# wjakob/nori

Hardware: AMD Instinct MI355X
Metric: Mrays/sec (primary+secondary) at 1024x1024 256spp (higher is better)
Workload: dtype f32; 1 GPU; pa4-cbox-path_mis; generator=tests/golden/pa4-cbox-path_mis.npz (scenes/pa4/cbox/cbox-distributed.xml), integrator=path_mis, width=1024, height=1024, spp=256, triangles=7948, parallelism=single GPU, seed_mode=per_sample, engine=wavefront

## Files before the change

### nori_amd/csrc/device/wavefront.hip

```cpp
#include <hip/hip_runtime.h>

#include <algorithm>
#include <cstdio>
#include <cstdlib>
#include <string>
#include <type_traits>
#include <vector>

#ifdef NORI_LAB
#include "wf_experiments.h"
#else
#define NORI_EXP_Q_GLOBAL
#define NORI_EXP_Q_LDS
#define NORI_EXP_Q_ALU
#define NORI_PROF_DECL
#define NORI_PROF_MARK(acc)
#define NORI_PROF_STORE
#define NORI_PROF_REPORT(h, k)
#define NORI_LAB_SHADE_PAD
#define NORI_LAB_SHADE_VERTEX
#define NORI_LAB_SHADE_STORE
#endif

#include "film.h"
#include "ktimer.h"
#include "shade_tables.h"
#include "rt_path.h"
#include "wavefront.h"
#include "wf_records.h"

using namespace nrt;

namespace {

constexpr int kB = 256;

enum { C_N = 0, C_HEAD = 2, C_OVERFLOW = 4, C_TAIL_HEAD = 5, C_SAMPLE = 6, C_HEAD_FRESH = 8, C_COUNT = 12 };
enum { S_CAM = 0, S_CLOSEST = 1, S_SHADOW = 2, S_NODES = 3, S_TRIS = 4, S_INVALID = 5, S_COUNT = 8 };
enum { Z_TRIPS = 0, Z_INNER_TRIPS = 1, Z_INNER_LANES = 2, Z_LEAF_TRIPS = 3, Z_LEAF_LANES = 4, Z_REFILLS = 5, Z_REFILL_LANES = 6, Z_COUNT = 8 };

constexpr uint32_t kShadeChunk = 4096u;

struct WfState {
    P3 *o;
    f4 *dA;
    f4 *dB;
    f4 *T_eta, *L_pdf;
    P3 *Ld;
    uint32_t *sidx;
    unsigned long long *rng;
};

struct WfBuf {
    WfState st[2];
    f4 *hit;
    f2 *samp_pos;
    P3 *samp_L;
    uint32_t *ctr;
    unsigned long long *stats;
    uint32_t capacity;
    int *stack_spill;
    unsigned long long *census;
};

struct WfBatch {
    uint32_t tile_first, n_tiles;
    uint32_t s_first, n_spp;
    uint32_t tile_mod, tile_rem, tiles_x;
    int32_t tile_w;
    int32_t inner_repeat;
    uint32_t flags;
    uint32_t pool;
};

enum { kStoredOnly = 0, kFreshOnly = 1, kMixed = 2 };
struct PassShape { uint32_t n_s, s0, n_fresh, n_f0, n; };
template <int MODE> __device__ __forceinline__ PassShape pass_shape(const uint32_t *ctr, int cur, const WfBatch &bt) {
    PassShape ps;
    ps.n_s = ctr[C_N + cur];
    ps.s0 = ctr[C_SAMPLE + cur];
    ps.n_f0 = (ps.n_s + 255u) & ~255u;
    const uint32_t total = bt.n_tiles * 256u * bt.n_spp;
    ps.n_fresh = MODE == kStoredOnly ? 0u : min(total - ps.s0, bt.pool > ps.n_f0 ? bt.pool - ps.n_f0 : 0u);
    ps.n = ps.n_fresh ? ps.n_f0 + ps.n_fresh : ps.n_s;
    return ps;
}
constexpr uint32_t kBatchNoAsmLoop = 1u;
constexpr uint32_t kBatchCountQ = 2u;

template <int DEPTH, bool SPILL, int BLOCK = kB>
struct LdsStackW {
    int *base; int sp;
    int *spill; uint32_t spill_stride;
    __device__ __forceinline__ void init(char *smem, int *spill_, uint32_t stride_) {
        base = reinterpret_cast<int *>(smem) + threadIdx.x; sp = 0; spill = spill_; spill_stride = stride_;
    }
    __device__ __forceinline__ void reset() { sp = 0; }
    __device__ __forceinline__ void push(int v) {
        if (sp < DEPTH) base[sp * BLOCK] = v;
        else spill[(size_t) (sp - DEPTH) * spill_stride + blockIdx.x * BLOCK + threadIdx.x] = v;
        sp++;
    }
    __device__ __forceinline__ int pop_or(int empty_value) {
        if (sp == 0) return empty_value;
        sp--;
        if (sp < DEPTH) return base[sp * BLOCK];
        return spill[(size_t) (sp - DEPTH) * spill_stride + blockIdx.x * BLOCK + threadIdx.x];
    }
    static constexpr int kLdsEntries = DEPTH;
};

typedef __attribute__((address_space(3))) int lds_int_t;
__device__ __forceinline__ uint32_t lds_address(const void *generic) {
    return (uint32_t) reinterpret_cast<uintptr_t>((const __attribute__((address_space(3))) char *) generic);
}
__device__ __forceinline__ lds_int_t *lds_int_at(uint32_t address) { return reinterpret_cast<lds_int_t *>(address); }

template <int DEPTH, int BLOCK>
struct LdsStackW<DEPTH, false, BLOCK> {
    uint32_t top;
    uint32_t wave_base;
    __device__ __forceinline__ void init(char *smem, int *, uint32_t) {
        wave_base = (uint32_t) __builtin_amdgcn_readfirstlane((int) (lds_address(smem) + (threadIdx.x & ~63u) * 4u)); top = 0u;
    }
    __device__ __forceinline__ void reset() {
        uint32_t lane;
        asm volatile("v_mbcnt_lo_u32_b32 %0, -1, 0\n\tv_mbcnt_hi_u32_b32 %0, -1, %0" : "=v"(lane));
        const uint32_t base = wave_base + lane * 4u;
        *lds_int_at(base) = kTravDone; top = base + BLOCK * 4u;
    }
    __device__ __forceinline__ void push(int v) { *lds_int_at(top) = v; top += BLOCK * 4u; }
    __device__ __forceinline__ int pop_or(int) { top -= BLOCK * 4u; return *lds_int_at(top); }
    static constexpr int kLdsEntries = DEPTH + 1;
};
// ... 319 lines not shown
                }
            }
            chunk_pos += min(avail, (uint32_t) __popcll(fresh));
            nClosest += (uint32_t) __popcll(__ballot(startedA));
            if (kFresh) nCam += (uint32_t) __popcll(__ballot(startedCam));
            if (kStored) nShadow += (uint32_t) __popcll(__ballot(startedB));
        }
        if (__ballot(trav_active(tv)) == 0ull) {
            if (exhausted && __ballot((rid & 2u) != 0u) == 0ull) break;
            continue;
        }
        NORI_PROF_MARK(prof_refill)
        if (COUNT) zc[Z_TRIPS]++;
        if constexpr (ASM) {
            static_assert(!WIDE && !COUNT, "the hand-written node loop: BVH2 nodes as 32-B records");
            f3 qo = tv.o, qr = tv.rcp;
            asm volatile("" : "+v"(qo.x), "+v"(qo.y), "+v"(qo.z), "+v"(qr.x), "+v"(qr.y), "+v"(qr.z));
            NodeqRay R;
            nodeq_ray(sc.grid, qo, qr, R);
            uint32_t stack_limit = 0xffffffffu;
            if constexpr (SPILL) stack_limit = stack.limit;
            const bool full = bvh2q_node_loop_asm<BLOCK * 4, SPILL>(tv.node, stack.top, tv.hit.t, R, (int) f2u(qr.x) >> 31, (int) f2u(qr.y) >> 31, (int) f2u(qr.z) >> 31,
                                           sc.nodes_q, image_address, bt.inner_repeat, leaf_threshold,
                                           (!exhausted || __ballot((rid & 2u) != 0u) != 0ull) ? 64 - refill_threshold : -1, stack_limit);
            if (SPILL && full && trav_at_inner(tv)) trav_inner_step_q<false>(sc, stack, tv, tc, top_lds);
        } else
        do {
            if (COUNT) { const int ni = __popcll(__ballot(trav_at_inner(tv))); if (ni) { zc[Z_INNER_TRIPS]++; zc[Z_INNER_LANES] += (uint32_t) ni; } }
            if (trav_at_inner(tv)) {
                if (WIDE) trav_wide_step<COUNT>(sc, stack, tv, tc, top_lds);
                else if (COUNT && count_q) trav_inner_step_q<COUNT>(sc, stack, tv, tc, top_lds);
                else trav_inner_step<COUNT>(sc, stack, tv, tc, top_lds);
            }
        } while (__popcll(__ballot(trav_at_inner(tv))) >= bt.inner_repeat);
        NORI_PROF_MARK(prof_node)
        const bool atLeaf = trav_at_leaf(tv);
        const int nLeaf = __popcll(__ballot(atLeaf));
        const bool innerLeft = __ballot(trav_at_inner(tv)) != 0ull;
        if (COUNT && nLeaf && (nLeaf >= leaf_threshold || !innerLeft)) { zc[Z_LEAF_TRIPS]++; zc[Z_LEAF_LANES] += (uint32_t) nLeaf; }
        if (atLeaf && (nLeaf >= leaf_threshold || !innerLeft)) trav_leaf_step<COUNT, false>(sc, stack, tv, tc, top_lds);
        NORI_PROF_MARK(prof_leaf)
    }
    if (unsaved) st_f4<1>(&b.hit[rid >> 2], tv.any ? hit_pack_here(nullptr, tv.hit.tri != kNoHit) : hit_pack_here(&tv.hit, (rid & 1u) != 0u));
#ifdef NORI_LAB_WAVE_COUNTERS
    if (lane == 0) {
        if (nClosest) atomicAdd(&b.stats[S_CLOSEST], (unsigned long long) nClosest);
        if (nShadow) atomicAdd(&b.stats[S_SHADOW], (unsigned long long) nShadow);
        if (kFresh && nCam) atomicAdd(&b.stats[S_CAM], (unsigned long long) nCam);
    }
#else
    __syncthreads();
    uint32_t *s_sum = reinterpret_cast<uint32_t *>(smem);
    if (threadIdx.x < 4u) s_sum[threadIdx.x] = 0u;
    __syncthreads();
    if (lane == 0) {
        if (nClosest) atomicAdd(&s_sum[0], nClosest);
        if (nShadow) atomicAdd(&s_sum[1], nShadow);
        if (kFresh && nCam) atomicAdd(&s_sum[2], nCam);
    }
    __syncthreads();
    if (threadIdx.x == 0) {
        if (s_sum[0]) atomicAdd(&b.stats[S_CLOSEST], (unsigned long long) s_sum[0]);
        if (s_sum[1]) atomicAdd(&b.stats[S_SHADOW], (unsigned long long) s_sum[1]);
        if (kFresh && s_sum[2]) atomicAdd(&b.stats[S_CAM], (unsigned long long) s_sum[2]);
    }
#endif
    if (COUNT) for (int off = 32; off > 0; off >>= 1) { tc.nodes += (uint32_t) __shfl_down((int) tc.nodes, off); tc.tris += (uint32_t) __shfl_down((int) tc.tris, off); }
    if (lane == 0) {
        if (COUNT) { atomicAdd(&b.stats[S_NODES], (unsigned long long) tc.nodes); atomicAdd(&b.stats[S_TRIS], (unsigned long long) tc.tris); }
        NORI_PROF_STORE
        if (COUNT && b.census) for (int k = 0; k < Z_COUNT; ++k) if (zc[k]) atomicAdd(&b.census[k], (unsigned long long) zc[k]);
    }
}

constexpr int kSB = 256;
static_assert(kSB == 256, "pass_shape starts the new paths of a pass at a multiple of 256");

__device__ __forceinline__ void shade_barrier() { asm volatile("s_waitcnt lgkmcnt(0)\n\ts_barrier" ::: "memory"); }

template <bool LDSTAB> struct ShadeTab { typedef SceneTables type; static __device__ __forceinline__ type make(const DevScene &sc, uint4 *) { type t = {&sc}; return t; } };
template <> struct ShadeTab<true> { typedef LdsTables type; static __device__ __forceinline__ type make(const DevScene &sc, uint4 *s_tab) { return shade_tables_copy(sc, s_tab); } };


#ifndef NORI_SHADE_WGS
#define NORI_SHADE_WGS 4
#endif
template <int INTEG, int MODE, bool LDSTAB, int MATSET>
__global__ __launch_bounds__(kSB, NORI_SHADE_WGS) void wf_shade(DevScene sc, WfBuf b, int cur, WfBatch bt) {
    NORI_LAB_SHADE_PAD
    const WfState S = b.st[cur], D = b.st[cur ^ 1];
    const uint32_t s_first = bt.s_first, n_spp = bt.n_spp;
    __shared__ uint4 s_tab[LDSTAB ? kShadeTabWords / 4 : 1];
    const typename ShadeTab<LDSTAB>::type tab = ShadeTab<LDSTAB>::make(sc, s_tab);
    constexpr bool kFresh = MODE != kStoredOnly, kStored = MODE != kFreshOnly;
    const PassShape shape = pass_shape<MODE>(b.ctr, cur, bt);
    const uint32_t n = shape.n, n_s = shape.n_s;
    const uint32_t rounds_total = (n + kSB - 1) / kSB;
    const uint32_t rounds_per_block = (rounds_total + gridDim.x - 1) / gridDim.x;
    const uint32_t r0 = blockIdx.x * rounds_per_block, r1 = min(rounds_total, r0 + rounds_per_block);
    const uint32_t r_mid = kStored ? min(r1, max(r0, shape.n_f0 / kSB)) : r0;
    __shared__ uint32_t s_wcnt[2][4], s_newbase;
    uint32_t out_base = 0u, out_used = 0u, out_len = 0u;
    bool overflow = false;
    const int wave = (int) (threadIdx.x >> 6), lane = lane_id();
    const uint32_t per_tile = 256u * n_spp;
    uint32_t pf_sidx = 0u; f4 pf_d, pf_L, pf_h;
    pf_d.x = pf_d.y = pf_d.z = pf_d.w = 0.0f; pf_L = pf_h = pf_d;
    auto round = [&](auto fresh_tag, uint32_t r, uint32_t r_end) {
        constexpr bool FRESH = decltype(fresh_tag)::value;
        const uint32_t i = r * kSB + threadIdx.x;
        bool survive = false;
        const uint32_t c_sidx = pf_sidx; const f4 c_d = pf_d, c_L = pf_L, c_h = pf_h;
        if (!FRESH && r + 1u < r_end && i + kSB < n_s) {
            pf_d = ld_f4<2>(&S.dA[i + kSB]); pf_sidx = ld_w<2>(&S.sidx[i + kSB]); pf_L = ld_f4<2>(&S.L_pdf[i + kSB]); pf_h = ld_f4<1>(&b.hit[i + kSB]);
        }
        f4 n_o, n_dA, n_dB, n_T, n_L, n_Ld;
        uint32_t n_fl = 0u, sidx = 0u;
        unsigned long long n_rng = 0ull;
        if (FRESH ? i < n : i < n_s) {
            uint32_t fl; f4 L4, d4, t4; Rng rng0; rng0.state = 0; rng0.inc = 0;
            if (FRESH) {
                f2 ps; RayIn cam;
                sidx = shape.s0 + (i - shape.n_f0);
                fl = first_vertex(sc, bt, sidx, ps, cam, rng0) ? (F_HAS_A | (2u << 4)) : 0u;
                L4.x = L4.y = L4.z = L4.w = 0.0f;
                t4.x = t4.y = t4.z = t4.w = 1.0f;
                d4.x = cam.d.x; d4.y = cam.d.y; d4.z = cam.d.z; d4.w = 0.0f;
            } else {
                d4 = c_d;
                fl = state_flags(d4);
            }
            if (fl & (F_HAS_A | F_HAS_B)) {
                if (!FRESH) { sidx = c_sidx; L4 = c_L; }
                const f4 h = FRESH ? ld_f4<1>(&b.hit[i]) : c_h;
                const uint32_t hw = __float_as_uint(h.w);
                bool done = false;
                NORI_LAB_SHADE_VERTEX
                if (fl & F_HAS_B) {
                    if (!(hw & kOccludedB)) {
                        const P3 ld = ld_p3<2>(&S.Ld[i]);
                        L4.x = L4.x + ld.x; L4.y = L4.y + ld.y; L4.z = L4.z + ld.z;
                    }
                    if (fl & F_END_AFTER_B) done = true;
                }
                PathState st;
                st.L = mk3(L4.x, L4.y, L4.z);
                if (!done) {
                    if (!FRESH) t4 = ld_f4<2>(&S.T_eta[i]);
                    Hit hit; bool found;
                    hit_unpack(sc, h, hit, found);
                    const uint32_t sl = (sidx % per_tile) >> 8;
                    uint64_t rng_state = rng0.state;
                    if (!FRESH) rng_state = ld_w<2>(&S.rng[i]);
                    vertex_unpack(st, fl, L4, t4, rng_state, ((uint64_t) (s_first + sl) << 1u) | 1u);
                    done = path_on_closest<INTEG, typename ShadeTab<LDSTAB>::type, MATSET>(sc, tab, st, hit, found, mk3(d4.x, d4.y, d4.z));
                    if (!done) {
                        survive = true;
                        vertex_pack(st, n_o, n_dA, n_dB, n_T, n_L, n_Ld, n_fl);
                        n_rng = st.rng.state;
                    }
                }
                if (done) {
                    P3 out; out.x = st.L.x; out.y = st.L.y; out.z = st.L.z;
                    st_p3<2>(&b.samp_L[sidx], out);
                }
            }
        }
        const unsigned long long mask = __ballot(survive);
        if (lane == 0) s_wcnt[r & 1u][wave] = (uint32_t) __popcll(mask);
        shade_barrier();
        const uint32_t c0 = s_wcnt[r & 1u][0], c1 = kSB > 64 ? s_wcnt[r & 1u][1] : 0u, c2 = kSB > 128 ? s_wcnt[r & 1u][2] : 0u, c3 = kSB > 192 ? s_wcnt[r & 1u][3] : 0u;
        const uint32_t c = c0 + c1 + c2 + c3;
        uint32_t off = (uint32_t) __popcll(mask & ((1ull << lane) - 1ull));
        off += wave > 0 ? c0 : 0u; off += wave > 1 ? c1 : 0u; off += wave > 2 ? c2 : 0u;
        const uint32_t room = out_len - out_used;
        uint32_t new_base = 0u, want = 0u;
        if (c > room) {
            const uint32_t expect = c * (r1 - r);
            want = r + 1u == r1 ? c - room : min(kShadeChunk, max(c - room, ((expect + expect / 8u + 63u) & ~63u) - min(room, expect)));
            if (threadIdx.x == 0) s_newbase = atomicAdd(&b.ctr[C_N + (cur ^ 1)], want);
            shade_barrier();
            new_base = s_newbase;
            if (new_base + want > b.capacity) overflow = true;
        }
        if (survive && !overflow) {
            const uint32_t j = off < room ? out_base + out_used + off : new_base + (off - room);
            st_p3<2>(&D.o[j], p3_of(n_o)); st_f4<2>(&D.T_eta[j], n_T); st_f4<2>(&D.L_pdf[j], n_L);
            st_f4<2>(&D.dA[j], state_dA(n_dA, n_fl, (n_fl & F_HAS_A) != 0u)); st_w<2>(&D.rng[j], n_rng); st_w<2>(&D.sidx[j], sidx);
            if (n_fl & F_HAS_B) { st_f4<2>(&D.dB[j], n_dB); st_p3<2>(&D.Ld[j], p3_of(n_Ld)); }
            NORI_LAB_SHADE_STORE
        }
        if (c > room) { out_base = new_base; out_used = c - room; out_len = want; }
        else out_used += c;
    };
    if (kStored) {
        if (r0 < r_mid && r0 * kSB + threadIdx.x < n_s) {
            const uint32_t i0 = r0 * kSB + threadIdx.x;
            pf_d = ld_f4<2>(&S.dA[i0]); pf_sidx = ld_w<2>(&S.sidx[i0]); pf_L = ld_f4<2>(&S.L_pdf[i0]); pf_h = ld_f4<1>(&b.hit[i0]);
        }
        for (uint32_t r = r0; r < r_mid; ++r) round(std::false_type(), r, r_mid);
    }
    if (kFresh) for (uint32_t r = r_mid; r < r1; ++r) round(std::true_type(), r, r1);
    for (uint32_t k = out_used + threadIdx.x; k < out_len; k += kSB) { f4 z; z.x = z.y = z.z = z.w = 0.0f; D.dA[out_base + k] = z; }
    if (overflow && threadIdx.x == 0) b.ctr[C_OVERFLOW] = 1u;
}

template <int INTEG, int MATSET = kAnyBsdf>
__global__ __launch_bounds__(kB) void wf_finish(DevScene sc, WfBuf b, int cur, WfBatch bt, int count) {
    extern __shared__ __attribute__((aligned(16))) char smem[];
    LdsStackW<16, true> stack;
    stack.init(smem, b.stack_spill, gridDim.x * kB);
    __shared__ uint4 s_tab[kShadeTabWords / 4];
    shade_tables_to_lds(sc, s_tab);
    const WfState S = b.st[cur];
    const uint32_t n = b.ctr[C_N + cur];
    const uint32_t per_tile = 256u * bt.n_spp;
    uint32_t nClosest = 0, nShadow = 0;
    TraversalCounters tc; tc.nodes = 0; tc.tris = 0;
    bool have = false, dry = false;
    uint32_t sidx = 0u, fl = 0u;
    f4 o, dA, dB, T, L, Ld;
    o.x = o.y = o.z = o.w = 0.0f; dA = dB = T = L = Ld = o;
    unsigned long long rng_state = 0ull;
    while (true) {
        const unsigned long long want = __ballot(!have && !dry);
        if (want != 0ull) {
            uint32_t base = 0u;
            if (lane_id() == 0) base = atomicAdd(&b.ctr[C_TAIL_HEAD], (uint32_t) __popcll(want));
            base = (uint32_t) __builtin_amdgcn_readfirstlane((int) base);
            const uint32_t i = base + __builtin_amdgcn_mbcnt_hi((uint32_t) (want >> 32), __builtin_amdgcn_mbcnt_lo((uint32_t) want, 0u));
            if (!have && !dry) {
                if (i >= n) dry = true;
                else {
                    dA = S.dA[i];
                    fl = state_flags(dA);
                    if (fl & (F_HAS_A | F_HAS_B)) {
                        have = true;
                        sidx = S.sidx[i]; dB = S.dB[i]; T = S.T_eta[i]; L = S.L_pdf[i];
                        const P3 o3 = S.o[i], l3 = S.Ld[i];
                        o.x = o3.x; o.y = o3.y; o.z = o3.z; o.w = kStoredMint; Ld.x = l3.x; Ld.y = l3.y; Ld.z = l3.z; Ld.w = 0.0f;
                        dA.w = kInf;
                        rng_state = S.rng[i];
                    }
                }
            }
        }
        if (__ballot(have) == 0ull) { if (__ballot(!dry) == 0ull) break; continue; }
        if (have) {
            bool fin = false;
            if (fl & F_HAS_B) {
                RayIn ray; ray.o = mk3(o.x, o.y, o.z); ray.d = mk3(dB.x, dB.y, dB.z); ray.mint = kEpsilon; ray.maxt = dB.w;
                Hit sh; ++nShadow;
                if (!traverse<true>(sc, ray, true, stack, sh, tc)) { L.x = L.x + Ld.x; L.y = L.y + Ld.y; L.z = L.z + Ld.z; }
                fin = (fl & F_END_AFTER_B) != 0u;
            }
            if (!fin) {
                RayIn ray; ray.o = mk3(o.x, o.y, o.z); ray.d = mk3(dA.x, dA.y, dA.z); ray.mint = o.w; ray.maxt = dA.w;
                Hit hit; ++nClosest;
                const bool found = traverse<true>(sc, ray, false, stack, hit, tc);
                if (found) hit.mesh = f2u(sc.shade_tris[(size_t) hit.tri * kShadeQuads].w);
                PathState st;
                vertex_unpack(st, fl, L, T, rng_state, ((uint64_t) (bt.s_first + ((sidx % per_tile) >> 8)) << 1u) | 1u);
                fin = path_on_closest<INTEG, MATSET>(sc, st, hit, found, ray.d);
                L.x = st.L.x; L.y = st.L.y; L.z = st.L.z;
                if (!fin) { vertex_pack(st, o, dA, dB, T, L, Ld, fl); rng_state = st.rng.state; }
            }
            if (fin) { P3 out; out.x = L.x; out.y = L.y; out.z = L.z; b.samp_L[sidx] = out; have = false; }
        }
    }
    for (int off = 32; off > 0; off >>= 1) {
        nClosest += (uint32_t) __shfl_down((int) nClosest, off);
        nShadow += (uint32_t) __shfl_down((int) nShadow, off);
        tc.nodes += (uint32_t) __shfl_down((int) tc.nodes, off); tc.tris += (uint32_t) __shfl_down((int) tc.tris, off);
    }
    __shared__ uint32_t s_sum[4];
    __syncthreads();
    if (threadIdx.x < 4u) s_sum[threadIdx.x] = 0u;
    __syncthreads();
    if (lane_id() == 0) {
        if (nClosest) atomicAdd(&s_sum[0], nClosest);
        if (nShadow) atomicAdd(&s_sum[1], nShadow);
        if (count) { atomicAdd(&s_sum[2], tc.nodes); atomicAdd(&s_sum[3], tc.tris); }
    }
    __syncthreads();
    if (threadIdx.x == 0) {
        if (s_sum[0]) atomicAdd(&b.stats[S_CLOSEST], (unsigned long long) s_sum[0]);
        if (s_sum[1]) atomicAdd(&b.stats[S_SHADOW], (unsigned long long) s_sum[1]);
        if (count) { atomicAdd(&b.stats[S_NODES], (unsigned long long) s_sum[2]); atomicAdd(&b.stats[S_TRIS], (unsigned long long) s_sum[3]); }
    }
}

__global__ __launch_bounds__(kB) void wf_tail_copy(WfBuf b, int cur, WfState D, uint32_t *d_ctr) {
    const WfState S = b.st[cur];
    const uint32_t n = b.ctr[C_N + cur];
    for (uint32_t i = blockIdx.x * kB + threadIdx.x; i < n; i += gridDim.x * kB) {
        D.o[i] = S.o[i]; D.dA[i] = S.dA[i]; D.dB[i] = S.dB[i]; D.T_eta[i] = S.T_eta[i]; D.L_pdf[i] = S.L_pdf[i]; D.Ld[i] = S.Ld[i];
        D.sidx[i] = S.sidx[i]; D.rng[i] = S.rng[i];
    }
    if (blockIdx.x == 0 && threadIdx.x == 0) { d_ctr[C_N] = n; d_ctr[C_TAIL_HEAD] = 0u; }
}

constexpr int kShadeGridMax = 4096;
#ifndef NORI_SPLIT_CUS_DEFAULT
#define NORI_SPLIT_CUS_DEFAULT 0
#endif
constexpr int kSplitCusDefault = NORI_SPLIT_CUS_DEFAULT;
constexpr size_t kSplitMinSamples = (size_t) 1 << 24;

int shade_grid(size_t paths) { return (int) std::min<size_t>(kShadeGridMax, std::max<size_t>(64, (paths + kShadeChunk - 1) / kShadeChunk)); }

size_t state_capacity(size_t paths) {
    return paths + (size_t) kShadeChunk * (size_t) shade_grid(paths) * (size_t) (kB / kSB) + 1024;
}

struct Pool {
    std::vector<void *> allocs;
    size_t capacity = 0;
    size_t bytes = 0;
    WfBuf buf;
    uint32_t *h_ctr = nullptr;
    int *spill = nullptr;
    size_t spill_ints = 0;
    void release() {
        for (void *p : allocs) (void) hipFree(p);
        allocs.clear(); capacity = 0; bytes = 0;
        if (spill) { (void) hipFree(spill); spill = nullptr; spill_ints = 0; }
        if (h_ctr) { (void) hipHostFree(h_ctr); h_ctr = nullptr; }
    }
};

#define WF_TRY(expr) do { hipError_t e__ = (expr); if (e__ != hipSuccess) return std::string(#expr) + ": " + hipGetErrorString(e__); } while (0)

template <class T> std::string pool_alloc(Pool &pool, T **out, size_t count) {
    void *p = nullptr;
    WF_TRY(hipMalloc(&p, std::max<size_t>(count * sizeof(T), 16)));
    pool.allocs.push_back(p); pool.bytes += count * sizeof(T);
    *out = reinterpret_cast<T *>(p);
    return std::string();
}

constexpr size_t kStateBytesPerRecord = 2 * (4 * sizeof(f4) + 2 * sizeof(P3) + sizeof(uint32_t) + sizeof(unsigned long long)) + sizeof(f4);

std::string ensure_pool(Pool &pool, size_t records) {
    if (pool.capacity >= records) return std::string();
    pool.release();
    WfBuf &b = pool.buf;
    std::string e;
#define A(field, count) if (!(e = pool_alloc(pool, &b.field, (count))).empty()) { pool.release(); return e; }
    for (int k = 0; k < 2; ++k) {
        A(st[k].o, records); A(st[k].dA, records); A(st[k].dB, records);
        A(st[k].T_eta, records); A(st[k].L_pdf, records); A(st[k].Ld, records);
        A(st[k].sidx, records); A(st[k].rng, records);
    }
    A(hit, records);
    A(ctr, (size_t) 2 * C_COUNT); A(stats, (size_t) 2 * S_COUNT);
#undef A
    WF_TRY(hipHostMalloc((void **) &pool.h_ctr, 2 * C_COUNT * sizeof(uint32_t)));
    pool.capacity = records;
    return std::string();
}

constexpr int kExtendBlockBvh2 = 1024, kExtendBlockWide = kB;
constexpr int kExtendWgsBvh2 = 2048 / kExtendBlockBvh2, kExtendWgsWide = 7, kExtendWgsWideFirst = 5;
constexpr size_t kLdsPerCu = 160 * 1024;
template <int STACK, bool SPILL, bool COUNT, int MODE>
void launch_extend(const DevScene &sc, const WfBuf &b, int cur, int refill, int grid, const WfBatch &bt, hipStream_t s) {
    const size_t image = (size_t) std::max(1u, sc.top_image_quads) * sizeof(f4);
    if (sc.wide) {
        const size_t lds = (size_t) LdsStackW<STACK, SPILL, kExtendBlockWide>::kLdsEntries * kExtendBlockWide * sizeof(int) + image;
        if (SPILL) hipLaunchKernelGGL((wf_extend<STACK, true, COUNT, MODE, true, false, kExtendBlockWide>), dim3(grid), dim3(kExtendBlockWide), lds, s, sc, b, cur, refill, bt);
    } else {
        constexpr bool kAsm = !COUNT;
        const bool use_asm = kAsm && sc.nodes_q != nullptr && sc.n_triangles < (1u << 25) && (bt.flags & kBatchNoAsmLoop) == 0u;
        const bool image_q = use_asm || (COUNT && (bt.flags & kBatchCountQ) != 0u);
        const size_t lds = (use_asm ? (size_t) ExtendStack<STACK, SPILL, kAsm, kExtendBlockBvh2>::type::kLdsEntries : (size_t) LdsStackW<STACK, SPILL, kExtendBlockBvh2>::kLdsEntries) *
                               kExtendBlockBvh2 * sizeof(int) + (size_t) std::max(1u, image_q ? sc.top_image_q_quads : sc.top_image_quads) * sizeof(f4);
        if (use_asm)
            hipLaunchKernelGGL((wf_extend<STACK, SPILL, COUNT, MODE, false, kAsm, kExtendBlockBvh2>), dim3(grid), dim3(kExtendBlockBvh2), lds, s, sc, b, cur, refill, bt);
        else
            hipLaunchKernelGGL((wf_extend<STACK, SPILL, COUNT, MODE, false, false, kExtendBlockBvh2>), dim3(grid), dim3(kExtendBlockBvh2), lds, s, sc, b, cur, refill, bt);
    }
}

void launch_extend_dyn(const DevScene &sc, const WfBuf &b, int cur, int refill, int lds_stack, bool spill, bool count, int mode,
                       int grid, const WfBatch &bt, hipStream_t s) {
#define G(S, P, C) if (mode == kFreshOnly) launch_extend<S, P, C, kFreshOnly>(sc, b, cur, refill, grid, bt, s); \
                   else launch_extend<S, P, C, kStoredOnly>(sc, b, cur, refill, grid, bt, s)
#define E(S, P) if (count) { G(S, P, true); } else { G(S, P, false); }
#define F(S) if (spill) { E(S, true); } else { E(S, false); }
    if (lds_stack <= 16) { F(16); } else if (lds_stack <= 24) { F(24); } else { F(32); }
#undef F
#undef E
#undef G
}

void launch_shade(const DevScene &sc, const WfBuf &b, int cur, const WfBatch &bt, int mode, int grid_, hipStream_t s) {
    const dim3 grid(grid_ * (kB / kSB)), block(kSB);
    const bool lds_tables = shade_tables_fit(sc);
    int matset = sc.integrator.type < INT_WHITTED ? kAnyBsdf : sc.bsdf_mask == 1u ? 1 : (sc.bsdf_mask & 8u) == 0u ? 7 : kAnyBsdf;
    if (getenv("NORI_HIP_SHADE_ANY_BSDF")) matset = kAnyBsdf;
    if (sc.integrator.type >= INT_WHITTED && sc.textured) matset = kAnyBsdf | kTextured;
    switch (sc.integrator.type) {
#define SH3(I, F, M) if (lds_tables) hipLaunchKernelGGL((wf_shade<I, F, true, M>), grid, block, 0, s, sc, b, cur, bt); \
                     else hipLaunchKernelGGL((wf_shade<I, F, false, M>), grid, block, 0, s, sc, b, cur, bt)
#define SH2(I, F) if (matset == 1) { SH3(I, F, 1); } else if (matset == 7) { SH3(I, F, 7); } else if (matset == kAnyBsdf) { SH3(I, F, kAnyBsdf); } \
                  else { SH3(I, F, kAnyBsdf | kTextured); }
#define SH1(I, F) SH3(I, F, kAnyBsdf)
#define SH(I, W) case I: if (mode == kFreshOnly) { W(I, kFreshOnly); } else if (mode == kMixed) { W(I, kMixed); } else { W(I, kStoredOnly); } break;
        SH(0, SH1) SH(1, SH1) SH(2, SH1) SH(3, SH2) SH(4, SH2) SH(5, SH2) SH(6, SH2)
#undef SH
#undef SH1
#undef SH2
#undef SH3
    }
}

void launch_finish(const DevScene &sc, const WfBuf &b, int cur, const WfBatch &bt, bool count, int grid_, hipStream_t s) {
    const dim3 grid(grid_), block(kB);
    const size_t lds = (size_t) LdsStackW<16, true>::kLdsEntries * kB * sizeof(int);
    switch (sc.integrator.type) {
#define FN(I) case I: hipLaunchKernelGGL((wf_finish<I>), grid, block, lds, s, sc, b, cur, bt, (int) count); break;
#define FNT(I) case I: if (sc.textured) { hipLaunchKernelGGL((wf_finish<I, kAnyBsdf | kTextured>), grid, block, lds, s, sc, b, cur, bt, (int) count); } \
                       else { hipLaunchKernelGGL((wf_finish<I>), grid, block, lds, s, sc, b, cur, bt, (int) count); } break;
        FN(0) FN(1) FN(2) FNT(3) FNT(4) FNT(5) FNT(6)
#undef FNT
#undef FN
    }
}

}

namespace nrt {

int wf_top_capacity(bool wide_nodes, bool records_32b, bool deeper_than_lds_stack) {
    const size_t per_wg = kLdsPerCu / (wide_nodes ? kExtendWgsWide : kExtendWgsBvh2);
    const size_t stacks = (size_t) (deeper_than_lds_stack && records_32b ? 18 : 17) * (wide_nodes ? kExtendBlockWide : kExtendBlockBvh2) * sizeof(int);
    const int stride = records_32b ? kTopStrideQuadsQ : kTopStrideQuads;
    int n = 0;
    while (n < kTopMaxNodes && stacks + (size_t) top_image_quads(n + 1, stride) * sizeof(f4) <= per_wg) ++n;
    return n;
}


struct WfEngine {
    Pool pool;
    hipStream_t streams[2] = {nullptr, nullptr};
    hipEvent_t events[3] = {nullptr, nullptr, nullptr};
    int n_cus = 0;
    hipStream_t split_streams[2] = {nullptr, nullptr};
    int split_cus = 0;
    hipEvent_t pipe_events[2][2] = {{nullptr, nullptr}, {nullptr, nullptr}};
    struct TailSide {
        WfState st; uint32_t *ctr = nullptr; size_t capacity = 0; std::vector<void *> allocs;
        int *spill = nullptr; size_t spill_ints = 0;
        void release() { for (void *q : allocs) (void) hipFree(q); allocs.clear(); capacity = 0; ctr = nullptr; if (spill) { (void) hipFree(spill); spill = nullptr; spill_ints = 0; } }
    } tail;
    hipEvent_t tail_events[3] = {nullptr, nullptr, nullptr};
    hipStream_t tail_stream = nullptr;
    int tail_stream_cus = 0;
};

bool ensure_tail_stream(WfEngine &e, int cus) {
    if (e.tail_stream && e.tail_stream_cus == cus) return true;
    if (e.tail_stream) { (void) hipStreamDestroy(e.tail_stream); e.tail_stream = nullptr; e.tail_stream_cus = 0; }
    if (cus < 8 || cus >= e.n_cus) return false;
    const uint32_t words = (uint32_t) ((e.n_cus + 31) / 32);
    std::vector<uint32_t> mask(words, 0u);
    for (int i = 0; i < cus; ++i) mask[(size_t) i / 32] |= 1u << (i % 32);
    if (hipExtStreamCreateWithCUMask(&e.tail_stream, words, mask.data()) != hipSuccess) { (void) hipGetLastError(); e.tail_stream = nullptr; return false; }
    e.tail_stream_cus = cus;
    return true;
}

std::string ensure_tail_side(WfEngine &e, size_t records, size_t spill_ints) {
    WfEngine::TailSide &t = e.tail;
    if (t.capacity < records) {
        t.release();
#define A(field, T) { void *q = nullptr; WF_TRY(hipMalloc(&q, records * sizeof(T))); t.allocs.push_back(q); t.st.field = reinterpret_cast<T *>(q); }
        A(o, P3) A(dA, f4) A(dB, f4) A(T_eta, f4) A(L_pdf, f4) A(Ld, P3) A(sidx, uint32_t) A(rng, unsigned long long)
#undef A
        { void *q = nullptr; WF_TRY(hipMalloc(&q, C_COUNT * sizeof(uint32_t))); t.allocs.push_back(q); t.ctr = reinterpret_cast<uint32_t *>(q); }
        t.capacity = records;
    }
    if (t.spill_ints < spill_ints) {
        if (t.spill) (void) hipFree(t.spill);
        t.spill = nullptr; t.spill_ints = 0;
        WF_TRY(hipMalloc((void **) &t.spill, spill_ints * sizeof(int)));
        t.spill_ints = spill_ints;
    }
    for (hipEvent_t &ev : e.tail_events) if (!ev) WF_TRY(hipEventCreateWithFlags(&ev, hipEventDisableTiming));
    return std::string();
}

bool ensure_split_streams(WfEngine &e, int cus) {
    if (e.split_cus == cus && e.split_streams[0] && e.split_streams[1]) return true;
    for (hipStream_t &st : e.split_streams) if (st) { (void) hipStreamDestroy(st); st = nullptr; }
    e.split_cus = 0;
    const int rows_total = e.n_cus / 8, rows = cus / 8;
    if (rows < 1 || rows >= rows_total) return false;
    const uint32_t words = (uint32_t) ((e.n_cus + 31) / 32);
    std::vector<uint32_t> shade(words, 0u), extend(words, 0u);
    std::vector<char> taken((size_t) rows_total, 0);
    for (int j = 0; j < rows; ++j) taken[(size_t) ((long long) j * rows_total / rows)] = 1;
    for (int i = 0; i < e.n_cus; ++i) {
        const bool in_row = i / 8 < rows_total && taken[(size_t) (i / 8)];
        (in_row ? shade : extend)[(size_t) i / 32] |= 1u << (i % 32);
    }
    if (hipExtStreamCreateWithCUMask(&e.split_streams[0], words, extend.data()) != hipSuccess ||
        hipExtStreamCreateWithCUMask(&e.split_streams[1], words, shade.data()) != hipSuccess) {
        (void) hipGetLastError();
        for (hipStream_t &st : e.split_streams) if (st) { (void) hipStreamDestroy(st); st = nullptr; }
        return false;
    }
    e.split_cus = cus;
    return true;
}

WfEngine *wavefront_create() {
    WfEngine *e = new WfEngine();
    int dev = 0; hipDeviceProp_t prop;
    if (hipGetDevice(&dev) == hipSuccess && hipGetDeviceProperties(&prop, dev) == hipSuccess) e->n_cus = prop.multiProcessorCount;
    if (e->n_cus <= 0) e->n_cus = 256;
    return e;
}

void wavefront_destroy(WfEngine *e) {
    if (!e) return;
    e->pool.release();
    for (hipStream_t &st : e->streams) if (st) { (void) hipStreamDestroy(st); st = nullptr; }
    for (hipStream_t &st : e->split_streams) if (st) { (void) hipStreamDestroy(st); st = nullptr; }
    for (hipEvent_t &ev : e->events) if (ev) { (void) hipEventDestroy(ev); ev = nullptr; }
    for (auto &pe : e->pipe_events) for (hipEvent_t &ev : pe) if (ev) { (void) hipEventDestroy(ev); ev = nullptr; }
    for (hipEvent_t &ev : e->tail_events) if (ev) { (void) hipEventDestroy(ev); ev = nullptr; }
    if (e->tail_stream) { (void) hipStreamDestroy(e->tail_stream); e->tail_stream = nullptr; }
    e->tail.release();
    delete e;
}

bool wavefront_excursions(unsigned long long out[4], bool reset) {
#if defined(NORI_COUNT_EXCURSIONS)
    unsigned long long h[4] = {0, 0, 0, 0};
    if (hipMemcpyFromSymbol(h, HIP_SYMBOL(g_nori_excursions), sizeof(h)) != hipSuccess) return false;
    for (int k = 0; k < 4; ++k) out[k] += h[k];
    if (reset) { const unsigned long long z[4] = {0, 0, 0, 0}; (void) hipMemcpyToSymbol(HIP_SYMBOL(g_nori_excursions), z, sizeof(z)); }
    return true;
#else
    (void) out; (void) reset;
    return false;
#endif
}

size_t wavefront_bytes_per_path() { return kStateBytesPerRecord; }
size_t wavefront_bytes_per_sample() { return 2 * (sizeof(f2) + sizeof(P3)); }
void wavefront_release_pool(WfEngine *e) { if (e) { e->pool.release(); e->tail.release(); } }

size_t wavefront_held_bytes(const WfEngine *e, const FilmStore &film) {
    return (e ? e->pool.bytes : 0) + film.capacity * (sizeof(f2) + sizeof(P3));
}

struct Pipe {
    hipStream_t stream = nullptr;
    hipStream_t extend_stream = nullptr;
    hipEvent_t ev_extend = nullptr, ev_shade = nullptr;
    WfBuf b;
    FilmStore film;
    uint32_t *h_ctr = nullptr;
    uint32_t tile_lo = 0, tile_hi = 0;
    uint32_t tiles_b = 0, spp_b = 0;
    uint32_t t0 = 0, s0 = 0;
    bool active = false, finished = false;
    int mode = kFreshOnly;
    uint32_t batch_samples = 0;
    uint32_t batch_rounds = 0;
    WfBatch bt;
    int cur = 0;
};

static WfBuf slice(const WfBuf &b, size_t off, size_t records, int k) {
    WfBuf v = b;
    for (int c = 0; c < 2; ++c) {
        WfState &t = v.st[c];
        t.o += off; t.dA += off; t.dB += off; t.T_eta += off; t.L_pdf += off; t.Ld += off;
        t.sidx += off; t.rng += off;
    }
    v.hit += off;
    v.ctr += (size_t) k * C_COUNT; v.stats += (size_t) k * S_COUNT;
    v.capacity = (uint32_t) records;
    return v;
}

std::string wavefront_render(WfEngine &eng, FilmStore &film_store, const DevScene &sc, const float *d_filter_table, const WfLaunch &L,
                             float *d_rgbw, void *stream_, WfStats &stats) {
    hipStream_t s = (hipStream_t) stream_;
    Pool &g_pool = eng.pool;
    hipStream_t (&g_streams)[2] = eng.streams;
    hipEvent_t (&g_events)[3] = eng.events;
    stats = WfStats();
    if (L.n_sel_tiles == 0 || L.spp_count == 0) return std::string();

    int n_pipes = 1;
    if (const char *e = getenv("NORI_HIP_WF_PIPES")) n_pipes = std::min(2, std::max(1, atoi(e)));
    int split_cus = kSplitCusDefault;
    if (const char *e = getenv("NORI_HIP_WF_SPLIT_CUS")) split_cus = std::max(0, atoi(e)) & ~7;
    if (getenv("NORI_HIP_WF_PIPES")) split_cus = 0;
    size_t split_min = kSplitMinSamples;
    if (const char *e = getenv("NORI_HIP_WF_SPLIT_MIN")) split_min = (size_t) std::max(0ll, atoll(e));
    if (L.n_sel_tiles < 2 || (size_t) L.n_sel_tiles * 256 * L.spp_count < split_min || L.film_reference || L.count_traversal) split_cus = 0;
    if (L.n_sel_tiles < 2 || (size_t) L.n_sel_tiles * 256 * L.spp_count < ((size_t) 1 << 22)) n_pipes = 1;
    if (split_cus >= eng.n_cus) split_cus = 0;
    if (split_cus > 0 && ensure_split_streams(eng, split_cus)) n_pipes = 2; else split_cus = 0;
    const bool split = split_cus > 0;

    const size_t budget = std::min<size_t>(std::max<size_t>(std::max(L.max_samples, L.max_paths) / n_pipes, 256), (size_t) 1 << 31);
    Pipe pipes[2];
    size_t need[2] = {0, 0};
    for (int k = 0; k < n_pipes; ++k) {
        Pipe &P = pipes[k];
        P.tile_lo = (uint32_t) ((uint64_t) L.n_sel_tiles * k / n_pipes);
        P.tile_hi = (uint32_t) ((uint64_t) L.n_sel_tiles * (k + 1) / n_pipes);
        const uint32_t nt = P.tile_hi - P.tile_lo;
        if ((size_t) nt * 256 > budget) { P.tiles_b = (uint32_t) (budget / 256); P.spp_b = 1; }
        else { P.tiles_b = nt; P.spp_b = (uint32_t) std::min<size_t>(L.spp_count, std::max<size_t>(1, budget / ((size_t) nt * 256))); }
        need[k] = (size_t) P.tiles_b * 256 * P.spp_b;
        P.t0 = P.tile_lo; P.s0 = 0;
    }
    int tail_cus = 32;
    if (const char *e = getenv("NORI_HIP_WF_TAIL_CUS")) tail_cus = std::max(0, atoi(e)) & ~7;
    {
        const Pipe &P0 = pipes[0];
        const uint64_t nt0 = P0.tile_hi - P0.tile_lo;
        const uint64_t batches = ((nt0 + P0.tiles_b - 1) / std::max(1u, P0.tiles_b)) * ((L.spp_count + P0.spp_b - 1) / std::max(1u, P0.spp_b));
        if (n_pipes != 1 || split || batches < 2 || L.film_reference || L.count_traversal || tail_cus >= eng.n_cus) tail_cus = 0;
        if (getenv("NORI_HIP_WF_FINISH") && atoi(getenv("NORI_HIP_WF_FINISH")) == 0) tail_cus = 0;
        if (tail_cus > 0 && !ensure_tail_stream(eng, tail_cus)) tail_cus = 0;
    }
    const bool overlap = tail_cus > 0;
    if (L.film_reference && (n_pipes != 1 || pipes[0].tiles_b != L.n_sel_tiles || pipes[0].spp_b != L.spp_count || L.tile_mod != 1))
        return "wavefront: film_order = reference needs the whole frame in one batch (tile_mod 1, wavefront_samples >= pixels x samples)";
    const size_t per_pipe = std::max(need[0], need[1]);
    size_t pool_paths = std::min(per_pipe, std::max<size_t>(L.max_paths / n_pipes, 256));
    if (const char *e = getenv("NORI_HIP_WF_POOL")) pool_paths = std::min(per_pipe, (size_t) std::max(256ll, atoll(e)));
    const size_t records = state_capacity(pool_paths);
    const int sh_grid = shade_grid(pool_paths);
    if (records >= ((size_t) 1 << 30)) return "wavefront: wavefront_paths too large (state index is 30 bits)";
    std::string err = ensure_pool(g_pool, records * n_pipes);
    if (!err.empty()) return err;
    FilmStore film;
    err = film_prepare(film_store, per_pipe * (overlap ? 2 : n_pipes), L.n_sel_tiles, L.tile_w, s, film);
    if (!err.empty()) return err;
    stats.state_bytes = g_pool.bytes + per_pipe * (overlap ? 2 : n_pipes) * (sizeof(f2) + sizeof(P3));
    WF_TRY(hipMemsetAsync(g_pool.buf.stats, 0, 2 * S_COUNT * sizeof(unsigned long long), s));

    for (int k = 0; k < 3; ++k) if (!g_events[k]) WF_TRY(hipEventCreateWithFlags(&g_events[k], hipEventDisableTiming));
    for (int k = 0; k < n_pipes; ++k) {
        Pipe &P = pipes[k];
        if (split) {
            P.extend_stream = eng.split_streams[0]; P.stream = eng.split_streams[1];
            for (hipEvent_t &ev : eng.pipe_events[k]) if (!ev) WF_TRY(hipEventCreateWithFlags(&ev, hipEventDisableTiming));
            P.ev_extend = eng.pipe_events[k][0]; P.ev_shade = eng.pipe_events[k][1];
        } else if (n_pipes == 1 && !overlap) P.stream = P.extend_stream = s;
        else {
            if (!g_streams[k]) WF_TRY(hipStreamCreateWithFlags(&g_streams[k], hipStreamNonBlocking));
            P.stream = P.extend_stream = g_streams[k];
        }
        P.b = slice(g_pool.buf, records * k, records, k);
        P.film = film; P.film.pos += per_pipe * k; P.film.L += per_pipe * k;
// ... 241 lines not shown
```

Before: 16710 Mrays/s.

## Keep path radiance in sample buffer and pack sidx with material pdf

Removes the per-record L_pdf f4 array from the wavefront path state. Accumulated radiance now lives in samp_L, indexed by sample, and is read and written only when a vertex actually adds light (emitter hit or unoccluded shadow contribution). The sample index and material pdf are packed into one 64-bit word. This cuts state bytes per record and per-round stream traffic, at the cost of scattered samp_L reads and writes plus an extra mesh-flag lookup to decide whether an emitter is hit.

```diff
diff --git a/nori_amd/csrc/device/wavefront.hip b/nori_amd/csrc/device/wavefront.hip
--- a/nori_amd/csrc/device/wavefront.hip
+++ b/nori_amd/csrc/device/wavefront.hip
@@ -45,11 +45,14 @@
     P3 *o;
     f4 *dA;
     f4 *dB;
-    f4 *T_eta, *L_pdf;
+    f4 *T_eta;
     P3 *Ld;
-    uint32_t *sidx;
+    unsigned long long *sidx_pdf;
     unsigned long long *rng;
 };
+__device__ __forceinline__ unsigned long long sidx_pdf_pack(uint32_t sidx, float pdf_mat) { return (unsigned long long) sidx | ((unsigned long long) __float_as_uint(pdf_mat) << 32); }
+__device__ __forceinline__ uint32_t sidx_of(unsigned long long sp) { return (uint32_t) sp; }
+__device__ __forceinline__ float pdf_mat_of(unsigned long long sp) { return __uint_as_float((uint32_t) (sp >> 32)); }
 
 struct WfBuf {
     WfState st[2];
@@ -535,6 +538,7 @@
 template <> struct ShadeTab<true> { typedef LdsTables type; static __device__ __forceinline__ type make(const DevScene &sc, uint4 *s_tab) { return shade_tables_copy(sc, s_tab); } };
 
 
+
 #ifndef NORI_SHADE_WGS
 #define NORI_SHADE_WGS 4
 #endif
@@ -557,15 +561,15 @@
     bool overflow = false;
     const int wave = (int) (threadIdx.x >> 6), lane = lane_id();
     const uint32_t per_tile = 256u * n_spp;
-    uint32_t pf_sidx = 0u; f4 pf_d, pf_L, pf_h;
-    pf_d.x = pf_d.y = pf_d.z = pf_d.w = 0.0f; pf_L = pf_h = pf_d;
+    unsigned long long pf_sp = 0ull; f4 pf_d, pf_h;
+    pf_d.x = pf_d.y = pf_d.z = pf_d.w = 0.0f; pf_h = pf_d;
     auto round = [&](auto fresh_tag, uint32_t r, uint32_t r_end) {
         constexpr bool FRESH = decltype(fresh_tag)::value;
         const uint32_t i = r * kSB + threadIdx.x;
         bool survive = false;
-        const uint32_t c_sidx = pf_sidx; const f4 c_d = pf_d, c_L = pf_L, c_h = pf_h;
+        const unsigned long long c_sp = pf_sp; const f4 c_d = pf_d, c_h = pf_h;
         if (!FRESH && r + 1u < r_end && i + kSB < n_s) {
-            pf_d = ld_f4<2>(&S.dA[i + kSB]); pf_sidx = ld_w<2>(&S.sidx[i + kSB]); pf_L = ld_f4<2>(&S.L_pdf[i + kSB]); pf_h = ld_f4<1>(&b.hit[i + kSB]);
+            pf_d = ld_f4<2>(&S.dA[i + kSB]); pf_sp = ld_w<2>(&S.sidx_pdf[i + kSB]); pf_h = ld_f4<1>(&b.hit[i + kSB]);
         }
         f4 n_o, n_dA, n_dB, n_T, n_L, n_Ld;
         uint32_t n_fl = 0u, sidx = 0u;
@@ -584,10 +588,18 @@
                 fl = state_flags(d4);
             }
             if (fl & (F_HAS_A | F_HAS_B)) {
-                if (!FRESH) { sidx = c_sidx; L4 = c_L; }
                 const f4 h = FRESH ? ld_f4<1>(&b.hit[i]) : c_h;
                 const uint32_t hw = __float_as_uint(h.w);
                 bool done = false;
+                bool adds = FRESH || ((fl & F_HAS_B) && !(hw & kOccludedB));
+                if (!FRESH) {
+                    sidx = sidx_of(c_sp);
+                    if (!((fl & F_HAS_B) && (fl & F_END_AFTER_B)) && (hw & kMissA) != kMissA)
+                        adds = adds || (tab.mesh(f2u(sc.shade_tris[(size_t) (hw & kMissA) * kShadeQuads].w)).flags & kMeshEmitter) != 0u;
+                    P3 c_L; c_L.x = c_L.y = c_L.z = 0.0f;
+                    if (adds) c_L = ld_p3<2>(&b.samp_L[sidx]);
+                    L4.x = c_L.x; L4.y = c_L.y; L4.z = c_L.z; L4.w = pdf_mat_of(c_sp);
+                }
                 NORI_LAB_SHADE_VERTEX
                 if (fl & F_HAS_B) {
                     if (!(hw & kOccludedB)) {
@@ -613,9 +625,9 @@
                         n_rng = st.rng.state;
                     }
                 }
-                if (done) {
+                {
                     P3 out; out.x = st.L.x; out.y = st.L.y; out.z = st.L.z;
-                    st_p3<2>(&b.samp_L[sidx], out);
+                    if (adds) st_p3<2>(&b.samp_L[sidx], out);
                 }
             }
         }
@@ -638,8 +650,8 @@
         }
         if (survive && !overflow) {
             const uint32_t j = off < room ? out_base + out_used + off : new_base + (off - room);
-            st_p3<2>(&D.o[j], p3_of(n_o)); st_f4<2>(&D.T_eta[j], n_T); st_f4<2>(&D.L_pdf[j], n_L);
-            st_f4<2>(&D.dA[j], state_dA(n_dA, n_fl, (n_fl & F_HAS_A) != 0u)); st_w<2>(&D.rng[j], n_rng); st_w<2>(&D.sidx[j], sidx);
+            st_p3<2>(&D.o[j], p3_of(n_o)); st_f4<2>(&D.T_eta[j], n_T);
+            st_f4<2>(&D.dA[j], state_dA(n_dA, n_fl, (n_fl & F_HAS_A) != 0u)); st_w<2>(&D.rng[j], n_rng); st_w<2>(&D.sidx_pdf[j], sidx_pdf_pack(sidx, n_L.w));
             if (n_fl & F_HAS_B) { st_f4<2>(&D.dB[j], n_dB); st_p3<2>(&D.Ld[j], p3_of(n_Ld)); }
             NORI_LAB_SHADE_STORE
         }
@@ -649,7 +661,7 @@
     if (kStored) {
         if (r0 < r_mid && r0 * kSB + threadIdx.x < n_s) {
             const uint32_t i0 = r0 * kSB + threadIdx.x;
-            pf_d = ld_f4<2>(&S.dA[i0]); pf_sidx = ld_w<2>(&S.sidx[i0]); pf_L = ld_f4<2>(&S.L_pdf[i0]); pf_h = ld_f4<1>(&b.hit[i0]);
+            pf_d = ld_f4<2>(&S.dA[i0]); pf_sp = ld_w<2>(&S.sidx_pdf[i0]); pf_h = ld_f4<1>(&b.hit[i0]);
         }
         for (uint32_t r = r0; r < r_mid; ++r) round(std::false_type(), r, r_mid);
     }
@@ -689,7 +701,10 @@
                     fl = state_flags(dA);
                     if (fl & (F_HAS_A | F_HAS_B)) {
                         have = true;
-                        sidx = S.sidx[i]; dB = S.dB[i]; T = S.T_eta[i]; L = S.L_pdf[i];
+                        const unsigned long long sp = S.sidx_pdf[i];
+                        sidx = sidx_of(sp); dB = S.dB[i]; T = S.T_eta[i];
+                        const P3 L3 = b.samp_L[sidx];
+                        L.x = L3.x; L.y = L3.y; L.z = L3.z; L.w = pdf_mat_of(sp);
                         const P3 o3 = S.o[i], l3 = S.Ld[i];
                         o.x = o3.x; o.y = o3.y; o.z = o3.z; o.w = kStoredMint; Ld.x = l3.x; Ld.y = l3.y; Ld.z = l3.z; Ld.w = 0.0f;
                         dA.w = kInf;
@@ -747,8 +762,8 @@
     const WfState S = b.st[cur];
     const uint32_t n = b.ctr[C_N + cur];
     for (uint32_t i = blockIdx.x * kB + threadIdx.x; i < n; i += gridDim.x * kB) {
-        D.o[i] = S.o[i]; D.dA[i] = S.dA[i]; D.dB[i] = S.dB[i]; D.T_eta[i] = S.T_eta[i]; D.L_pdf[i] = S.L_pdf[i]; D.Ld[i] = S.Ld[i];
-        D.sidx[i] = S.sidx[i]; D.rng[i] = S.rng[i];
+        D.o[i] = S.o[i]; D.dA[i] = S.dA[i]; D.dB[i] = S.dB[i]; D.T_eta[i] = S.T_eta[i]; D.Ld[i] = S.Ld[i];
+        D.sidx_pdf[i] = S.sidx_pdf[i]; D.rng[i] = S.rng[i];
     }
     if (blockIdx.x == 0 && threadIdx.x == 0) { d_ctr[C_N] = n; d_ctr[C_TAIL_HEAD] = 0u; }
 }
@@ -792,7 +807,8 @@
     return std::string();
 }
 
-constexpr size_t kStateBytesPerRecord = 2 * (4 * sizeof(f4) + 2 * sizeof(P3) + sizeof(uint32_t) + sizeof(unsigned long long)) + sizeof(f4);
+constexpr size_t kStateBytesPerRecord = 2 * (3 * sizeof(f4) + 2 * sizeof(P3) + 2 * sizeof(unsigned long long)) + sizeof(f4);
+static_assert(kStateBytesPerRecord == 2 * 88 + 16, "wf_records.h: 88 B per record and copy");
 
 std::string ensure_pool(Pool &pool, size_t records) {
     if (pool.capacity >= records) return std::string();
@@ -802,8 +818,8 @@
 #define A(field, count) if (!(e = pool_alloc(pool, &b.field, (count))).empty()) { pool.release(); return e; }
     for (int k = 0; k < 2; ++k) {
         A(st[k].o, records); A(st[k].dA, records); A(st[k].dB, records);
-        A(st[k].T_eta, records); A(st[k].L_pdf, records); A(st[k].Ld, records);
-        A(st[k].sidx, records); A(st[k].rng, records);
+        A(st[k].T_eta, records); A(st[k].Ld, records);
+        A(st[k].sidx_pdf, records); A(st[k].rng, records);
     }
     A(hit, records);
     A(ctr, (size_t) 2 * C_COUNT); A(stats, (size_t) 2 * S_COUNT);
@@ -930,7 +946,7 @@
     if (t.capacity < records) {
         t.release();
 #define A(field, T) { void *q = nullptr; WF_TRY(hipMalloc(&q, records * sizeof(T))); t.allocs.push_back(q); t.st.field = reinterpret_cast<T *>(q); }
-        A(o, P3) A(dA, f4) A(dB, f4) A(T_eta, f4) A(L_pdf, f4) A(Ld, P3) A(sidx, uint32_t) A(rng, unsigned long long)
+        A(o, P3) A(dA, f4) A(dB, f4) A(T_eta, f4) A(Ld, P3) A(sidx_pdf, unsigned long long) A(rng, unsigned long long)
 #undef A
         { void *q = nullptr; WF_TRY(hipMalloc(&q, C_COUNT * sizeof(uint32_t))); t.allocs.push_back(q); t.ctr = reinterpret_cast<uint32_t *>(q); }
         t.capacity = records;
@@ -1033,8 +1049,8 @@
     WfBuf v = b;
     for (int c = 0; c < 2; ++c) {
         WfState &t = v.st[c];
-        t.o += off; t.dA += off; t.dB += off; t.T_eta += off; t.L_pdf += off; t.Ld += off;
-        t.sidx += off; t.rng += off;
+        t.o += off; t.dA += off; t.dB += off; t.T_eta += off; t.Ld += off;
+        t.sidx_pdf += off; t.rng += off;
     }
     v.hit += off;
     v.ctr += (size_t) k * C_COUNT; v.stats += (size_t) k * S_COUNT;
```

Result: no change. 16570 Mrays/s (-0.8%).
